# lrmantovani10/Stable-Diffusion.mojo

Hardware: AMD Instinct MI355X
Metric: UNet denoising steps/sec @ 512x512 latent, batch=8 (higher is better)
Workload: dtype f16; 1 GPU; Tiny-SD UNet 512x512 (latent 4x64x64), batch 8/GPU, 50-step DDPM schedule, 77-token context, no CFG, random-init weights (BASELINE configs[1]); global_batch=8, parallelism=dp1 (independent prompts, weights broadcast once)

## Files before the change

### include/tsd.h

```cpp
#ifndef TSD_H
#define TSD_H

#include <stddef.h>
#include <stdint.h>

#ifdef __cplusplus
extern "C" {
#endif

#define TSD_VERSION 100

typedef enum tsd_status {
  TSD_OK = 0,
  TSD_E_ARG = -1,
  TSD_E_SHAPE = -2,
  TSD_E_ALLOC = -3,
  TSD_E_HIP = -4,
  TSD_E_RCCL = -5,
  TSD_E_STATE = -6,
  TSD_E_NONFINITE = -7
} tsd_status;

typedef struct tsd_ctx tsd_ctx;
typedef struct tsd_model tsd_model;
// ... 152 lines not shown
};
#define TSD_GD_VERSION_1 1
enum tsd_gemm_operand { TSD_GO_A0 = 0, TSD_GO_A1, TSD_GO_A2, TSD_GO_W, TSD_GO_WT1, TSD_GO_R, TSD_GO_BIAS, TSD_GO_ROWVEC, TSD_GO_C,
                        TSD_GO_VT, TSD_GO_GN, TSD_GO_COUNT };
int tsd_debug_gemm_record(tsd_ctx* ctx, int on);
int tsd_debug_gemm_recorded(tsd_ctx* ctx, int i, int64_t* desc, int n);
int tsd_debug_gemm_run(tsd_ctx* ctx, const int64_t* desc, int n, int cfg, const void* const* host_in, void* const* host_out,
                       int64_t* ext, int64_t* info);
int tsd_debug_model_fold(tsd_model* m, int block, void* wf, float* bf);
int tsd_debug_attn_bench(tsd_ctx* ctx, int B, int H, int d, int Sq, int Sk, int iters, float* ms);
int tsd_debug_attn_exact_passes(tsd_ctx* ctx, int reset);
int tsd_debug_set_attn_qb(tsd_ctx* ctx, int mode);
int tsd_debug_set_attn_diag(tsd_ctx* ctx, int on);
int tsd_debug_set_res_fuse_skip(tsd_ctx* ctx, int on);
int tsd_debug_set_qkv_fuse(tsd_ctx* ctx, int on);
int tsd_debug_mfma_sustained(tsd_ctx* ctx, float ms_target, float* tflops, float* clock_ghz);

double tsd_flop_count(int kind, int L, int T);

#ifdef __cplusplus
}
#endif
#endif
```

### stable-diffusion.mojo_amd/csrc/api_model.cpp

```cpp
#include <dlfcn.h>
#include <math.h>
#include <string.h>

#include <vector>

#include "graph.h"

#define NOTNULL(p) \
  if (!(p)) TSD_FAIL(TSD_E_ARG, "%s: argument '%s' is NULL", __func__, #p)

namespace {
int h2d(tsd_ctx* c, void* dst, const void* src, size_t bytes) {
  if (c->launch()) HIP_TRY(hipMemcpyAsync(dst, src, bytes, hipMemcpyHostToDevice, c->stream));
  return TSD_OK;
}
int d2h(tsd_ctx* c, void* dst, const void* src, size_t bytes) {
  if (c->launch()) HIP_TRY(hipMemcpyAsync(dst, src, bytes, hipMemcpyDeviceToHost, c->stream));
  return TSD_OK;
}
template <class F>
int run_model(tsd_model* m, F&& fn) {
  tsd_ctx* ctx = m->ctx;
  HIP_TRY(hipSetDevice(ctx->device));
  TSD_TRY(model_check_ready(m));
// ... 90 lines not shown
  tsd_model* dec = nullptr;
  tsd_ctx* ctx = nullptr;
  int B = 0, L = 0, T = 0, Tp = 0, cfg = 0;
  float cfg_scale = 7.5f;
  char* state = nullptr;
  float* latents = nullptr;
  float* lat2 = nullptr;
  half_t* ctx16 = nullptr;
  float* eps = nullptr;
  float* tdev = nullptr;
  float* temb = nullptr;
  float* noise = nullptr;
  float* images = nullptr;
  float* hist = nullptr;
  size_t noise_cap = 0;
  int n_train = 1000, n_infer = 50, start = 0;
  std::vector<float> alphas_cumprod;
  std::vector<int> timesteps;
  int sampler = TSD_SAMPLER_DDPM, spacing = TSD_SPACING_LEADING;
  float eta = 0.f;
  int hist_valid_for = -1;
  bool uploaded = false, has_noise = false;
  size_t plan_unet = 0, plan_dec = 0;
  unsigned opt_gen = 0;
  bool poisoned = false;
  bool decoded = false;
};

static bool host_all_finite(const float* p, size_t n) {
  unsigned bad = 0;
// ... 3 lines not shown
    bad |= ((u & 0x7f800000u) == 0x7f800000u);
  }
  return bad == 0;
}
#define SESSION_NOT_POISONED(s)                                                                                              \
  do {                                                                                                                       \
    if ((s)->poisoned)                                                                                                       \
      TSD_FAIL(TSD_E_NONFINITE, "session: inf / NaN was found in this session's latents or images (reported at an earlier " \
               "download); its state is unusable until upload() replaces it");                                              \
  } while (0)

static int build_schedule(tsd_session* s) {
  sampler_alphas_cumprod(s->n_train, s->alphas_cumprod);
  return sampler_timesteps(s->spacing, s->n_train, s->n_infer, s->start, s->timesteps);
}
static void schedule_changed(tsd_session* s) {
  s->uploaded = false; s->has_noise = false;
  s->hist_valid_for = -1;
  s->decoded = false;
}

extern "C" int tsd_session_create(tsd_model* diffusion, tsd_model* decoder, int B, int L, int T, int cfg,
                                  tsd_session** out) {
  NOTNULL(diffusion); NOTNULL(out);
  if (!is_diffusion_kind(diffusion->kind)) TSD_FAIL(TSD_E_ARG, "session: first model must be a Diffusion");
  if (decoder && (!is_decoder_kind(decoder->kind) || decoder->ctx != diffusion->ctx))
    TSD_FAIL(TSD_E_ARG, "session: decoder must be a Decoder on the same context");
  const int Bu = cfg ? 2 * B : B;
  if (B <= 0 || Bu > 16 || L <= 0 || L % 8 || T <= 0) TSD_FAIL(TSD_E_SHAPE, "session: B=%d (UNet batch %d <= 16) L=%d T=%d", B, Bu, L, T);
  tsd_ctx* ctx = diffusion->ctx;
// ... 14 lines not shown
  s->ctx16 = (half_t*)(s->state + o_ctx); s->eps = (float*)(s->state + o_eps);
  s->tdev = (float*)(s->state + o_t); s->temb = (float*)(s->state + o_te);
  s->images = decoder ? (float*)(s->state + o_img) : nullptr;
  s->hist = (float*)(s->state + o_hist);
  if (build_schedule(s) != TSD_OK) { hipFree(s->state); delete s; return TSD_E_ARG; }
  *out = s;
  return TSD_OK;
}

extern "C" int tsd_session_destroy(tsd_session* s) {
  if (!s) return TSD_OK;
  hipSetDevice(s->ctx->device);
  hipStreamSynchronize(s->ctx->stream);
  if (s->state) hipFree(s->state);
  if (s->noise) hipFree(s->noise);
  delete s;
  return TSD_OK;
}

extern "C" int tsd_session_set_schedule(tsd_session* s, int num_training_steps, int num_inference_steps,
                                        int start_step) {
  NOTNULL(s);
  if (num_training_steps <= 0 || num_inference_steps <= 0 || num_inference_steps > num_training_steps ||
      start_step < 0 || start_step >= num_inference_steps)
    TSD_FAIL(TSD_E_ARG, "schedule: train=%d infer=%d start=%d", num_training_steps, num_inference_steps, start_step);
  s->n_train = num_training_steps; s->n_infer = num_inference_steps; s->start = start_step;
  schedule_changed(s);
  return build_schedule(s);
}
extern "C" int tsd_session_set_sampler(tsd_session* s, int kind, float eta, int spacing) {
// ... 37 lines not shown
    const size_t bytes = s->timesteps.size() * nl * 4;
    if (bytes > s->noise_cap) {
      if (s->noise) HIP_TRY(hipFree(s->noise));
      s->noise = nullptr; s->noise_cap = 0;
      hipError_t e = hipMalloc((void**)&s->noise, bytes);
      if (e != hipSuccess) TSD_FAIL(TSD_E_ALLOC, "session: noise hipMalloc(%zu) failed", bytes);
      s->noise_cap = bytes;
    }
    HIP_TRY(hipMemcpyAsync(s->noise, noise, bytes, hipMemcpyHostToDevice, ctx->stream));
  }
  HIP_TRY(hipStreamSynchronize(ctx->stream));
  TSD_TRY(model_check_ready(s->unet));
  if (s->dec) TSD_TRY(model_check_ready(s->dec));
  Arena& a = ctx->arena;
  const int Bu = s->cfg ? 2 * B : B;
  a.planning = true; a.top = 0; a.peak = 0;
  int r = g_unet_forward(s->unet, s->lat2, s->ctx16, T, Tp, s->temb, Bu, L, s->eps);
  size_t need = a.peak;
  if (r == TSD_OK && s->dec) {
    a.top = 0; a.peak = 0;
    r = g_decoder_forward(s->dec, s->latents, B, L, s->images);
    need = std::max(need, a.peak);
  }
  a.planning = false; a.top = 0; a.peak = 0;
  if (r != TSD_OK) return r;
  TSD_TRY(ctx_reserve_arena(ctx, need));
  s->opt_gen = ctx->opt.gen;
  s->uploaded = true;
  s->poisoned = false;
  s->decoded = false;
  s->hist_valid_for = -1;
  return TSD_OK;
}

static void ddpm_coeffs(const tsd_session* s, int t, int prev, float* sa, float* sb, float* c_x0, float* c_xt, float* sigma) {
  const float a_t = s->alphas_cumprod[t];
  const float a_prev = prev >= 0 ? s->alphas_cumprod[prev] : 1.f;
  const float b_t = 1.f - a_t, b_prev = 1.f - a_prev;
  const float cur_a = a_t / a_prev, cur_b = 1.f - cur_a;
  *sa = sqrtf(a_t); *sb = sqrtf(b_t);
  *c_x0 = sqrtf(a_prev) * cur_b / b_t;
// ... 4 lines not shown
}

extern "C" int tsd_session_step(tsd_session* s, int i) {
  NOTNULL(s);
  if (!s->uploaded) TSD_FAIL(TSD_E_STATE, "session: upload() before step()");
  SESSION_NOT_POISONED(s);
  if (s->opt_gen != s->ctx->opt.gen) TSD_FAIL(TSD_E_STATE, "session: a tsd_debug_set_* call changed this context's options after upload() sized the workspace; upload() again");
  if (i < 0 || i >= (int)s->timesteps.size()) TSD_FAIL(TSD_E_ARG, "session: step %d out of range", i);
  tsd_ctx* ctx = s->ctx;
  const int B = s->B, L = s->L, Bu = s->cfg ? 2 * B : B;
  const size_t nl = (size_t)B * 4 * L * L;
  const int t = s->timesteps[i];
  const bool have_hist = s->sampler == TSD_SAMPLER_DPMPP_2M && s->hist_valid_for == i;
  s->hist_valid_for = -1;
  s->decoded = false;
  TSD_TRY(launch_time_embedding(ctx, nullptr, (float)t, Bu, s->temb));
  const float* lat_in = s->latents;
  if (s->cfg) {
    HIP_TRY(hipMemcpyAsync(s->lat2, s->latents, nl * 4, hipMemcpyDeviceToDevice, ctx->stream));
    HIP_TRY(hipMemcpyAsync(s->lat2 + nl, s->latents, nl * 4, hipMemcpyDeviceToDevice, ctx->stream));
    lat_in = s->lat2;
  }
  ctx->arena.top = 0;
  const bool eps_nhwc = s->unet->unet.final_conv.Opad == 4;
  TSD_TRY(g_unet_forward(s->unet, lat_in, s->ctx16, s->T, s->Tp, s->temb, Bu, L, s->eps, eps_nhwc));
  ctx->arena.top = 0;
  const float* eps_u = s->cfg ? s->eps + nl : nullptr;
  if (s->sampler == TSD_SAMPLER_DDPM) {
    float sa, sb, c_x0, c_xt, sigma;
    const int prev = s->spacing == TSD_SPACING_LEADING ? t - s->n_train / s->n_infer
                                                       : (i + 1 < (int)s->timesteps.size() ? s->timesteps[i + 1] : -1);
    ddpm_coeffs(s, t, prev, &sa, &sb, &c_x0, &c_xt, &sigma);
    const float* nz = (s->has_noise && t > 0) ? s->noise + (size_t)i * nl : nullptr;
    return launch_ddpm_step(ctx, s->latents, s->eps, eps_u, s->cfg_scale, nz, (int64_t)nl, sa, sb, c_x0, c_xt, sigma,
                            eps_nhwc ? L * L : 0);
  }
  double cd[8];
  TSD_TRY(sampler_coeffs(s->sampler, s->eta, s->alphas_cumprod, s->timesteps, i, have_hist ? 1 : 0, cd));
  const SamplerCoeffs c = {(float)cd[2], (float)cd[3], (float)cd[4], (float)cd[5], (float)cd[6], (float)cd[7]};
  const bool multistep = s->sampler == TSD_SAMPLER_DPMPP_2M;
// ... 160 lines not shown
```

### stable-diffusion.mojo_amd/csrc/common.h

```cpp
#pragma once
#include <hip/hip_runtime.h>
#include <stdint.h>
#include <stdio.h>
#include <string>
#include <vector>

#include "../../include/tsd.h"

typedef _Float16 half_t;

void tsd_set_error(const char* fmt, ...);
#define TSD_FAIL(code, ...)      \
  do {                           \
    tsd_set_error(__VA_ARGS__);  \
    return (code);               \
  } while (0)
#define HIP_TRY(expr)                                                                              \
  do {                                                                                             \
    hipError_t e__ = (expr);                                                                       \
    if (e__ != hipSuccess) TSD_FAIL(TSD_E_HIP, "%s failed: %s (%s:%d)", #expr, hipGetErrorString(e__), __FILE__, __LINE__); \
  } while (0)
#define TSD_TRY(expr)            \
  do {                           \
    int r__ = (expr);            \
// ... 11 lines not shown
    size_t n = a + bytes;
    if (n > peak) peak = n;
    if (!planning && n > cap) return nullptr;
    top = n;
    return planning ? (void*)(uintptr_t)(0x1000 + a) : (void*)(base + a);
  }
};

struct TsdOptions {
  int qkv_fuse = 1;
  int res_fuse_skip = 1;
  int gn_composite = 1;
  int conv_in_im2col = 1;
  int chain = 1;
  int fold_out = 1;
  int conv_w_tm_mib = 2, lin_w_tm = 1, lin_w_tm_kib = 1024;
  int attn_qb = 2;
  int attn_qb_force = 0;
  int attn_wg8 = 1;
  int attn8_var = 0;
  int attn_diag = 1;
  int attn_xcd = 0;
  int xcdn = 0, conv_halo = 0, splitk = 1, splitk_mink = 4096, splitk_tiles = 256, splitk_small = 8, splitk_wide = 1, splitk_ring4 = 0,
      splitk_big = 0, sk_cfg = 5, thin_cfg = 0, tune = 15, sk256 = 0, skip128 = 1;
  int force_cfg = -1;
  int sk_big_graph = 0;
  char cfg_override[512] = "";
  int gn_apply_mult = 2;
  int gn_finalize_min = 2048;
  int debug_occ = 0;
// ... 268 lines not shown
```

### stable-diffusion.mojo_amd/csrc/graph.cpp

```cpp
#include <math.h>

#include "graph.h"

#define CHECK_ALLOC(p) \
  if (!(p)) TSD_FAIL(TSD_E_ALLOC, "workspace arena exhausted (%s:%d)", __FILE__, __LINE__)

static int zero_async(tsd_ctx* ctx, void* p, size_t bytes) {
  if (!ctx->launch()) return TSD_OK;
  HIP_TRY(hipMemsetAsync(p, 0, bytes, ctx->stream));
  return TSD_OK;
}

Act act_alloc_gn(tsd_ctx* ctx, int B, int H, int W, int C, int groups) {
  Act a = act_alloc(ctx, B, H, W, C);
  if (a.p && groups > 0 && C % groups == 0) {
    a.gn_buf = arena_alloc<float>(ctx, (int64_t)B * ceil_div(H * W, 32) * groups * 2);
    a.gn_groups = a.gn_buf ? groups : 0;
  }
  return a;
}

static void gn_emit(const tsd_ctx* ctx, GemmArgs& g, Act* dst, int rows_per_sample) {
  if (!dst || !dst->gn_buf || dst->gn_groups <= 0 || g.N != dst->C || (g.epi & (EPI_OUT_F32 | EPI_GEGLU))) return;
  const int ns = gemm_gnstats_slabs(ctx, g.M, g.N, g.K, g.batch, g.conv, rows_per_sample, dst->gn_groups);
// ... 339 lines not shown
  half_t* ao = arena_alloc<half_t>(ctx, M * C); CHECK_ALLOC(ao);
  TSD_TRY(g_qkv_proj(ctx, h0, B, S, C, w.in_proj, qk, vt, S));
  AttnArgs fa;
  fa.Q = qk; fa.ldq = 2 * C; fa.sQ = (int64_t)S * 2 * C;
  fa.K = qk + C; fa.ldk = 2 * C; fa.sK = (int64_t)S * 2 * C;
  fa.Vt = vt; fa.ldvt = S; fa.sVt = (int64_t)C * S;
  fa.O = ao; fa.ldo = C; fa.sO = (int64_t)S * C;
  fa.B = B; fa.H = 1; fa.d = C; fa.Sq = S; fa.Sk = S; fa.scale = 1.f / sqrtf((float)C);
  TSD_TRY(g_attn_core(ctx, fa));
  CatSrc a; a.p0 = ao; a.ld0 = C; a.C0 = C;
  TSD_TRY(g_linear(ctx, a, M, w.out_proj.w, w.out_proj.Kpad, C, C, w.out_proj.b, x.p, x.ld, 0, out.p, out.ld, &out, S));
  ctx->arena.release(mark);
  return TSD_OK;
}

static int g_unet_full_forward(tsd_model* m, const float* latents_chw, const half_t* ctx16, int T, int Tp,
                               const float* temb, int B, int L, float* eps_out_chw, bool eps_nhwc);

int g_unet_forward(tsd_model* m, const float* latents_chw, const half_t* ctx16, int T, int Tp, const float* temb, int B,
                   int L, float* eps_out_chw, bool eps_nhwc) {
  if (is_full_unet_kind(m->kind)) {
    const int prev = gemm_set_splitk_big(m->ctx, 4);
    const int r = g_unet_full_forward(m, latents_chw, ctx16, T, Tp, temb, B, L, eps_out_chw, eps_nhwc);
    gemm_set_splitk_big(m->ctx, prev);
    return r;
  }
  tsd_ctx* ctx = m->ctx;
  const UNetW& u = m->unet;
  if (L % 8) TSD_FAIL(TSD_E_SHAPE, "UNet: latent side %d must be a multiple of 8", L);
  float* t1 = arena_alloc<float>(ctx, (int64_t)B * 1280); CHECK_ALLOC(t1);
  float* time = arena_alloc<float>(ctx, (int64_t)B * 1280); CHECK_ALLOC(time);
  float* tvec = arena_alloc<float>(ctx, (int64_t)B * u.tproj.N); CHECK_ALLOC(tvec);
  TSD_TRY(launch_small_linear(ctx, temb, B, 320, 320, u.t1.w, u.t1.Kpad, u.t1.b, 1280, 0, t1, 1280));
  TSD_TRY(launch_small_linear(ctx, t1, B, 1280, 1280, u.t2.w, u.t2.Kpad, u.t2.b, 1280, 1, time, 1280));
  TSD_TRY(launch_small_linear(ctx, time, B, 1280, 1280, u.tproj.w, u.tproj.Kpad, u.tproj.b, u.tproj.N, 1, tvec,
                              u.tproj.N));
  const int tld = u.tproj.N;
  const bool in_im2col = ctx->opt.conv_in_im2col && u.conv_in_im2col && u.conv1.I == 4;
  Act x0 = act_alloc(ctx, B, L, L, 64); CHECK_ALLOC(x0.p);
  if (in_im2col) TSD_TRY(launch_chw_f32_to_im2col3x3_f16(ctx, latents_chw, B, 4, L, L, x0.p));
  else TSD_TRY(launch_chw_f32_to_nhwc_f16(ctx, latents_chw, B, 4, L, L, 4, 1.f, x0.p, 64));
  Act a[24];
  auto alloc_out = [&](int i, int side, int C) -> int {
    const int groups = i == 23 ? 320 : (i == 11 ? concat_stat_groups(C, 640, 32) : (i == 16 ? concat_stat_groups(C, 320, 32) : 32));
    a[i] = act_alloc_gn(ctx, B, side, side, C, groups);
    CHECK_ALLOC(a[i].p);
    return TSD_OK;
  };
  const int L1 = L / 2, L2 = L / 4;
  auto res = [&](int i, const CatSrc& src, int side_in, int ups) -> int {
    const ResW& w = u.res[i - 1];
    TSD_TRY(alloc_out(i, ups ? side_in * 2 : side_in, w.cout));
    return g_resblock(ctx, src, B, side_in, side_in, ups, w, tvec, tld, a[i]);
  };
  const int CK = u.kproj_all.N;
  half_t* kc_all = arena_alloc<half_t>(ctx, (int64_t)B * Tp * CK); CHECK_ALLOC(kc_all);
  half_t* vtc_all = arena_alloc<half_t>(ctx, (int64_t)B * CK * Tp); CHECK_ALLOC(vtc_all);
  if (ctx_kv_fused_ok(ctx, u, Tp)) {
    GemmArgs g;
    g.A0 = ctx16; g.lda0 = u.kproj_all.Kpad; g.Wt = u.kproj_all.w; g.ldw = u.kproj_all.Kpad;
    g.M = B * Tp; g.N = 2 * CK; g.K = u.kproj_all.Kpad; g.C = kc_all; g.ldc = CK;
    if (u.kproj_all.w_tm) { g.Wt = u.kproj_all.w_tm; g.ldw = 64; g.w_kts = 2 * CK * 128; }
    g.Vt = vtc_all; g.vt_n0 = CK; g.vt_ld = Tp; g.vt_S = Tp; g.vt_sB = (int64_t)CK * Tp;
    TSD_TRY(launch_gemm(ctx, g));
  } else {
    GemmArgs g;
    g.A0 = ctx16; g.lda0 = u.kproj_all.Kpad; g.Wt = u.kproj_all.w; g.ldw = u.kproj_all.Kpad;
    g.M = B * Tp; g.N = CK; g.K = u.kproj_all.Kpad; g.C = kc_all; g.ldc = CK;
    TSD_TRY(launch_gemm(ctx, g));
    GemmArgs v;
    v.A0 = u.vproj_all.w; v.lda0 = u.vproj_all.Kpad; v.sA = 0;
    v.Wt = ctx16; v.ldw = u.vproj_all.Kpad; v.sW = (int64_t)Tp * u.vproj_all.Kpad;
    v.M = CK; v.N = Tp; v.K = u.vproj_all.Kpad; v.batch = B;
    v.C = vtc_all; v.ldc = Tp; v.sC = (int64_t)CK * Tp;
    TSD_TRY(launch_gemm(ctx, v));
  }
  auto attn = [&](int i) -> int {
    TSD_TRY(alloc_out(i, a[i - 1].H, a[i - 1].C));
    const AttnW& w = u.attn[i - 1];
    CtxKV kv;
    kv.K = kc_all + w.kv_off; kv.ldk = CK; kv.sK = (int64_t)Tp * CK;
    kv.Vt = vtc_all + (int64_t)w.kv_off * Tp; kv.ldvt = Tp; kv.sVt = (int64_t)CK * Tp;
    return g_unet_attn(ctx, a[i - 1], w, ctx16, T, Tp, a[i], &kv);
  };
  TSD_TRY(alloc_out(1, L, 320));
  if (in_im2col) TSD_TRY(g_linear(ctx, cat1(x0), (int64_t)B * L * L, u.conv_in_im2col, 64, u.conv1.Opad, 64, u.conv1.b, nullptr, 0, 0, a[1].p,
                                  a[1].ld, &a[1], L * L));
  else TSD_TRY(g_conv3x3(ctx, x0, u.conv1, 1, 1, 1, 0, nullptr, 0, nullptr, 0, false, a[1].p, a[1].ld, &a[1]));
  TSD_TRY(res(2, cat1(a[1]), L, 0));
  TSD_TRY(attn(3));
// ... 19 lines not shown
  TSD_TRY(attn(21));
  TSD_TRY(res(22, cat2(a[21], a[1]), L, 0));
  TSD_TRY(attn(23));
  Act hf = act_alloc(ctx, B, L, L, 320); CHECK_ALLOC(hf.p);
  TSD_TRY(launch_groupnorm(ctx, norm_src(cat1(a[23]), 320), B, L * L, 320, 320, 1e-5f, 1.f, 1, hf.p, hf.ld,
                           a[23].gn_groups == 320 ? a[23].gn_part : nullptr, a[23].gn_nslab));
  if (eps_nhwc && u.final_conv.Opad == 4)
    return g_conv3x3(ctx, hf, u.final_conv, 1, 1, 1, 0, nullptr, 0, nullptr, 0, true, eps_out_chw, 4);
  float* eps_tmp = arena_alloc<float>(ctx, (int64_t)B * L * L * 4); CHECK_ALLOC(eps_tmp);
  TSD_TRY(g_conv3x3(ctx, hf, u.final_conv, 1, 1, 1, 0, nullptr, 0, nullptr, 0, true, eps_tmp, 4));
  TSD_TRY(launch_nhwc_f32_to_chw_f32(ctx, eps_tmp, B, 4, L, L, 4, eps_out_chw));
  return TSD_OK;
}

static int g_unet_full_forward(tsd_model* m, const float* latents_chw, const half_t* ctx16, int T, int Tp,
                               const float* temb, int B, int L, float* eps_out_chw, bool eps_nhwc) {
  tsd_ctx* ctx = m->ctx;
  const UNetW& u = m->unet;
  if (L % 16) TSD_FAIL(TSD_E_SHAPE, "full-size UNet: latent side %d must be a multiple of 16", L);
  float* t1 = arena_alloc<float>(ctx, (int64_t)B * 1280); CHECK_ALLOC(t1);
  float* time = arena_alloc<float>(ctx, (int64_t)B * 1280); CHECK_ALLOC(time);
  float* tvec = arena_alloc<float>(ctx, (int64_t)B * u.tproj.N); CHECK_ALLOC(tvec);
  TSD_TRY(launch_small_linear(ctx, temb, B, 320, 320, u.t1.w, u.t1.Kpad, u.t1.b, 1280, 0, t1, 1280));
  TSD_TRY(launch_small_linear(ctx, t1, B, 1280, 1280, u.t2.w, u.t2.Kpad, u.t2.b, 1280, 1, time, 1280));
  TSD_TRY(launch_small_linear(ctx, time, B, 1280, 1280, u.tproj.w, u.tproj.Kpad, u.tproj.b, u.tproj.N, 1, tvec,
                              u.tproj.N));
  const int tld = u.tproj.N;
  const bool in_im2col = ctx->opt.conv_in_im2col && u.conv_in_im2col && !u.conv.empty() && u.conv[0].I == 4 && SD15_STEPS[0].l.kind == L_CONV &&
                         SD15_STEPS[0].l.d == 1;
  Act x0 = act_alloc(ctx, B, L, L, 64); CHECK_ALLOC(x0.p);
  if (in_im2col) TSD_TRY(launch_chw_f32_to_im2col3x3_f16(ctx, latents_chw, B, 4, L, L, x0.p));
  else TSD_TRY(launch_chw_f32_to_nhwc_f16(ctx, latents_chw, B, 4, L, L, 4, 1.f, x0.p, 64));
  const int CK = u.kproj_all.N;
  half_t* kc_all = arena_alloc<half_t>(ctx, (int64_t)B * Tp * CK); CHECK_ALLOC(kc_all);
  half_t* vtc_all = arena_alloc<half_t>(ctx, (int64_t)B * CK * Tp); CHECK_ALLOC(vtc_all);
  if (ctx_kv_fused_ok(ctx, u, Tp)) {
    GemmArgs g;
    g.A0 = ctx16; g.lda0 = u.kproj_all.Kpad; g.Wt = u.kproj_all.w; g.ldw = u.kproj_all.Kpad;
    g.M = B * Tp; g.N = 2 * CK; g.K = u.kproj_all.Kpad; g.C = kc_all; g.ldc = CK;
    if (u.kproj_all.w_tm) { g.Wt = u.kproj_all.w_tm; g.ldw = 64; g.w_kts = 2 * CK * 128; }
    g.Vt = vtc_all; g.vt_n0 = CK; g.vt_ld = Tp; g.vt_S = Tp; g.vt_sB = (int64_t)CK * Tp;
    TSD_TRY(launch_gemm(ctx, g));
  } else {
    GemmArgs g;
    g.A0 = ctx16; g.lda0 = u.kproj_all.Kpad; g.Wt = u.kproj_all.w; g.ldw = u.kproj_all.Kpad;
    g.M = B * Tp; g.N = CK; g.K = u.kproj_all.Kpad; g.C = kc_all; g.ldc = CK;
    TSD_TRY(launch_gemm(ctx, g));
    GemmArgs v;
    v.A0 = u.vproj_all.w; v.lda0 = u.vproj_all.Kpad; v.sA = 0;
    v.Wt = ctx16; v.ldw = u.vproj_all.Kpad; v.sW = (int64_t)Tp * u.vproj_all.Kpad;
    v.M = CK; v.N = Tp; v.K = u.vproj_all.Kpad; v.batch = B;
    v.C = vtc_all; v.ldc = Tp; v.sC = (int64_t)CK * Tp;
    TSD_TRY(launch_gemm(ctx, v));
  }
  std::vector<Act> skips;
  Act cur = x0;
  for (int i = 0; i < SD15_N; i++) {
    const UNetStep& st = SD15_STEPS[i];
    const LayerDef& l = st.l;
    const int next_groups = i == SD15_N - 1 ? u.final_groups : 32;
    auto stat_groups = [&](int C) -> int {
      if (i + 1 < SD15_N && SD15_STEPS[i + 1].l.kind == L_RES && (SD15_STEPS[i + 1].flags & U_POP) && !(st.flags & U_PUSH) && !skips.empty())
        return concat_stat_groups(C, skips.back().C, 32);
      return next_groups;
    };
    Act y;
    if (l.kind == L_CONV) {
      const int side = cur.H / l.d;
// ... 211 lines not shown
```

### stable-diffusion.mojo_amd/csrc/graph.h

```cpp
#pragma once
#include "model.h"

struct CatSrc {
  const half_t* p0 = nullptr; int ld0 = 0; int C0 = 0;
  const half_t* p1 = nullptr; int ld1 = 0; int C1 = 0;
  const float* gn_part0 = nullptr; int gn_nslab0 = 0, gn_groups0 = 0;
  const float* gn_part1 = nullptr; int gn_nslab1 = 0, gn_groups1 = 0;
};
static inline CatSrc cat1(const Act& a) {
  CatSrc c; c.p0 = a.p; c.ld0 = a.ld; c.C0 = a.C;
  c.gn_part0 = a.gn_part; c.gn_nslab0 = a.gn_nslab; c.gn_groups0 = a.gn_groups;
  return c;
}
static inline int concat_stat_groups(int C0, int C1, int groups) {
  if (C1 <= 0 || C1 % groups || (C0 + C1) % groups) return groups;
  const int cf = C1 / groups, cpg = (C0 + C1) / groups;
  return (cpg % cf == 0 && C0 % cf == 0 && C0 / cf <= 256) ? C0 / cf : groups;
}
Act act_alloc_gn(tsd_ctx* ctx, int B, int H, int W, int C, int groups);
static inline CatSrc cat2(const Act& a, const Act& b) {
  CatSrc c = cat1(a); c.p1 = b.p; c.ld1 = b.ld; c.C1 = b.C;
  c.gn_part1 = b.gn_part; c.gn_nslab1 = b.gn_nslab; c.gn_groups1 = b.gn_groups;
  return c;
}
// ... 6 lines not shown
             const half_t* res, int ldr, int epi_extra, void* y, int ldy, Act* stat = nullptr, int rows_per_sample = 0,
             const half_t* w_tm = nullptr);

int g_resblock(tsd_ctx* ctx, const CatSrc& x, int B, int Hin, int Win, int ups, const ResW& w, const float* tvec,
               int tld, Act& out);
struct CtxKV {
  const half_t* K = nullptr; int ldk = 0; int64_t sK = 0;
  const half_t* Vt = nullptr; int ldvt = 0; int64_t sVt = 0;
};
int g_unet_attn(tsd_ctx* ctx, const Act& x, const AttnW& w, const half_t* ctx16, int T, int Tp, Act& out,
                const CtxKV* pre = nullptr);
int g_vae_attn(tsd_ctx* ctx, const Act& x, const VaeAttnW& w, Act& out);
int g_attn_core(tsd_ctx* ctx, const AttnArgs& fa);
int g_qkv_proj(tsd_ctx* ctx, const half_t* x, int B, int S, int C, const LinW& in_proj, half_t* qk, half_t* vt, int Sp);

int g_unet_forward(tsd_model* m, const float* latents_chw, const half_t* ctx16, int T, int Tp, const float* temb, int B,
                   int L, float* eps_out_chw, bool eps_nhwc = false);
int g_decoder_forward(tsd_model* m, const float* latents_chw, int B, int L, float* images_chw);
int g_encoder_forward(tsd_model* m, const float* images_chw, const float* noise_chw, int B, int S, float* latents_chw);

template <class F>
int run_planned(tsd_ctx* ctx, F&& fn) {
  Arena& a = ctx->arena;
  a.planning = true; a.top = 0; a.peak = 0;
  int r = fn();
  a.planning = false;
  const size_t need = a.peak;
  a.top = 0; a.peak = 0;
  if (r != TSD_OK) return r;
  TSD_TRY(ctx_reserve_arena(ctx, need));
  r = fn();
  a.top = 0;
// ... 4 lines not shown
```

### stable-diffusion.mojo_amd/csrc/model.cpp

```cpp
#include <math.h>
#include <string.h>

#include "model.h"

bool attn_tail_weights_ok(const AttnW& w) {
  const int C = w.C;
  const bool plain = !w.ln[1].w && !w.ln[1].b && !w.ln[2].w && !w.ln[2].b && !w.gelu_erf;
  return plain && C == 320 && w.n_head == 8 && w.n_embed == 40 && w.sa_out.b && w.ca_out.b && w.geglu1.b && w.geglu2.b &&
         w.conv_out.b && !w.ca_q.b && w.sa_out.Kpad == C && w.ca_q.Kpad == C && w.ca_out.Kpad == C && w.geglu1.Kpad == C &&
         w.geglu2.Kpad == 4 * C && w.conv_out.Ipad == C && w.conv_out.k == 1;
}

bool attn_head_weights_ok(const AttnW& w) {
  const int C = w.C;
  return C == 320 && w.n_head == 8 && w.n_embed == 40 && !w.gn.w && !w.gn.b && !w.ln[0].w && !w.ln[0].b && w.conv_in.b &&
         w.conv_in.k == 1 && w.conv_in.Ipad == C && w.conv_in.Opad == C && !w.sa_in.b && w.sa_in.Kpad == C && w.sa_in.N == 3 * C;
}

static void model_invalidate_derived(tsd_model* m) {
  m->ready = false;
  for (auto& a : m->unet.attn) { a.tail_stream = nullptr; a.head_stream = nullptr; a.fold_w = nullptr; a.fold_w_tm = nullptr; a.fold_b = nullptr; }
  m->unet.conv_in_im2col = nullptr;
  m->vae.conv_in_im2col = nullptr;
  for (auto& r : m->unet.res) { r.conv1.w_tm = nullptr; r.conv2.w_tm = nullptr; }
  m->unet.conv4.w_tm = nullptr; m->unet.conv7.w_tm = nullptr; m->unet.kproj_all.w_tm = nullptr;
  for (auto& cv : m->unet.conv) cv.w_tm = nullptr;
  for (auto& a : m->unet.attn) {
    for (LinW* l : {&a.sa_in, &a.sa_out, &a.ca_q, &a.ca_out, &a.geglu1, &a.geglu2}) l->w_tm = nullptr;
    a.conv_in.w_tm = nullptr; a.conv_out.w_tm = nullptr;
  }
}

static size_t packed_bytes(const ParamSpec& p) {
  if (!p.used) return 0;
  switch (p.kind) {
// ... 487 lines not shown
```

### stable-diffusion.mojo_amd/csrc/model.h

```cpp
#pragma once
#include <map>
#include <string>
#include <vector>

#include "common.h"

enum ParamKind { P_CONV_W = 0, P_CONV_B = 1, P_LIN_W = 2, P_LIN_B = 3 };

struct ParamSpec {
  std::string name;
  int64_t shape[4] = {0, 0, 0, 0};
  int ndim = 0;
  int kind = 0;
  bool used = true;
  float bound = 0.f;
  float offset = 0.f;
  int Opad = 0, Kpad = 0;
  int interleave = 0;
  int region = 0;
  size_t off = 0, bytes = 0;
  int64_t numel() const {
    int64_t n = 1;
    for (int i = 0; i < ndim; i++) n *= shape[i];
    return n;
// ... 76 lines not shown
  ClipLayerW layer[12];
  NormAffine final_ln;
};

struct PlanKey { int B, L, T; bool operator<(const PlanKey& o) const { return B != o.B ? B < o.B : (L != o.L ? L < o.L : T < o.T); } };

struct tsd_model {
  tsd_ctx* ctx = nullptr;
  int kind = 0;
  std::vector<ParamSpec> params;
  std::map<std::string, int> index;
  char* blob = nullptr;
  size_t blob_bytes = 0;
  std::vector<char> loaded;
  bool ready = false;
  UNetW unet;
  VaeW vae;
  ClipW clip;
  std::map<PlanKey, size_t> plans;
  char* derived = nullptr;
  size_t derived_bytes = 0;
};

int model_resolve(tsd_model* m);
ConvW model_conv(const tsd_model* m, const std::string& prefix);
LinW model_lin(const tsd_model* m, const std::string& prefix, bool use_bias);
int model_check_ready(tsd_model* m);
```

### stable-diffusion.mojo_amd/csrc/runtime.cpp

```cpp
#include <stdarg.h>
#include <stdlib.h>
#include <string.h>

#include "common.h"

static thread_local char g_err[512] = "";

void tsd_set_error(const char* fmt, ...) {
  va_list ap;
  va_start(ap, fmt);
  vsnprintf(g_err, sizeof(g_err), fmt, ap);
  va_end(ap);
}

static int env_int(const char* name, int dflt) { const char* e = getenv(name); return e && *e ? atoi(e) : dflt; }
void options_from_env(TsdOptions& o) {
  o.qkv_fuse = env_int("TSD_QKV_FUSE", o.qkv_fuse);
  o.res_fuse_skip = env_int("TSD_RES_FUSE_SKIP", o.res_fuse_skip);
  o.gn_composite = env_int("TSD_GN_COMPOSITE", o.gn_composite);
  o.conv_in_im2col = env_int("TSD_CONV_IN_IM2COL", o.conv_in_im2col);
  o.chain = env_int("TSD_CHAIN", o.chain) ? 1 : 0;
  o.fold_out = env_int("TSD_FOLD_OUT", o.fold_out) ? 1 : 0;
  o.conv_w_tm_mib = env_int("TSD_CONV_W_TM", o.conv_w_tm_mib);
  o.lin_w_tm = env_int("TSD_LIN_W_TM", o.lin_w_tm);
  o.lin_w_tm_kib = env_int("TSD_LIN_W_TM_KIB", o.lin_w_tm_kib);
  { const int q = env_int("TSD_ATTN_QB", o.attn_qb); if (q == 1 || q == 2) o.attn_qb = q; }
  o.attn_xcd = env_int("TSD_ATTN_XCD", o.attn_xcd);
  o.attn_wg8 = env_int("TSD_ATTN_WG8", o.attn_wg8) ? 1 : 0;
  o.attn8_var = env_int("TSD_ATTN8_VAR", o.attn8_var);
  o.xcdn = env_int("TSD_GEMM_XCDN", o.xcdn);
  o.conv_halo = env_int("TSD_CONV_HALO", o.conv_halo);
  o.splitk = env_int("TSD_GEMM_SPLITK", o.splitk);
  o.splitk_mink = env_int("TSD_GEMM_SPLITK_MINK", o.splitk_mink);
  o.splitk_tiles = env_int("TSD_GEMM_SPLITK_TILES", o.splitk_tiles);
  o.splitk_small = env_int("TSD_GEMM_SPLITK_SMALL", o.splitk_small);
  o.splitk_wide = env_int("TSD_GEMM_SPLITK_WIDE", o.splitk_wide);
  o.splitk_ring4 = env_int("TSD_GEMM_SPLITK_RING4", o.splitk_ring4);
// ... 192 lines not shown
```

### stable-diffusion.mojo_amd/tsd/_lib.py

```python
import ctypes as C
import os

import numpy as np

_HERE = os.path.dirname(os.path.abspath(__file__))
LIB_PATH = os.environ.get("TSD_LIB") or os.path.join(os.path.dirname(_HERE), "lib", "libtsd.so")

TSD_OK, TSD_E_ARG, TSD_E_SHAPE, TSD_E_ALLOC, TSD_E_HIP, TSD_E_RCCL, TSD_E_STATE, TSD_E_NONFINITE = 0, -1, -2, -3, -4, -5, -6, -7
os.environ.setdefault("HIP_FORCE_DEV_KERNARG", "1")

MODEL_DIFFUSION, MODEL_DECODER, MODEL_ENCODER, MODEL_CLIP, MODEL_DIFFUSION_SD15, MODEL_DIFFUSION_SD15_TORCH = 1, 2, 3, 4, 5, 6
MODEL_CLIP_TORCH, MODEL_DECODER_TORCH, MODEL_ENCODER_TORCH = 7, 8, 9
SAMPLER_KINDS = {"ddpm": 0, "ddim": 1, "dpmpp_2m": 2}
TIMESTEP_SPACINGS = {"leading": 0, "trailing": 1}


def sampler_kind(kind):
    return SAMPLER_KINDS.get(kind.lower(), -1) if isinstance(kind, str) else int(kind)


def timestep_spacing(spacing):
    return TIMESTEP_SPACINGS.get(spacing.lower(), -1) if isinstance(spacing, str) else int(spacing)


# ... 81 lines not shown
        "tsd_dist_unique_id": ([vp], i), "tsd_dist_init": ([vp, i, i, vp], i),
        "tsd_dist_broadcast_weights": ([vp, i], i), "tsd_dist_finalize": ([vp], i),
        "tsd_dist_comm_count": ([vp, C.POINTER(i)], i),
        "tsd_flop_count": ([i, i, i], C.c_double),
        "tsd_debug_splitk_errors": ([vp], i),
        "tsd_debug_xcd_round_robin": ([], i),
        "tsd_debug_nonfinite_count": ([vp, i], i),
        "tsd_debug_set_fused_attention": ([vp, i], i),
        "tsd_debug_gemm_bench": ([vp, i, i, i, i, i, i, i, i, i, i, fp], i),
        "tsd_debug_attn_bench": ([vp, i, i, i, i, i, i, fp], i),
        "tsd_debug_attn_exact_passes": ([vp, i], i),
        "tsd_debug_set_attn_qb": ([vp, i], i),
        "tsd_debug_set_attn_diag": ([vp, i], i),
        "tsd_debug_set_res_fuse_skip": ([vp, i], i),
        "tsd_debug_set_qkv_fuse": ([vp, i], i),
        "tsd_debug_mfma_sustained": ([vp, C.c_float, fp, fp], i),
        "tsd_debug_gemm_check": ([vp, i, i, i, i, i, i, i, i, i, i, fp, fp], i),
        "tsd_debug_gemm_record": ([vp, i], i),
        "tsd_debug_gemm_recorded": ([vp, i, C.POINTER(i64), i], i),
        "tsd_debug_model_fold": ([vp, i, vp, fp], i),
        "tsd_debug_gemm_run": ([vp, C.POINTER(i64), i, i, C.POINTER(vp), C.POINTER(vp), C.POINTER(i64), C.POINTER(i64)], i),
    }
    for name, (args, res) in sig.items():
        fn = getattr(l, name)
        fn.argtypes = args
        fn.restype = res


EXPORTS = None

# ... 95 lines not shown
```

### stable-diffusion.mojo_amd/tsd/model.py

```python
import ctypes as C

import numpy as np

from . import _lib
from ._lib import check, f32, lib, ptr, sampler_kind, timestep_spacing, vp

KINDS = {"diffusion": _lib.MODEL_DIFFUSION, "decoder": _lib.MODEL_DECODER, "encoder": _lib.MODEL_ENCODER,
         "clip": _lib.MODEL_CLIP, "diffusion_sd15": _lib.MODEL_DIFFUSION_SD15,
         "diffusion_sd15_torch": _lib.MODEL_DIFFUSION_SD15_TORCH, "clip_torch": _lib.MODEL_CLIP_TORCH,
         "decoder_torch": _lib.MODEL_DECODER_TORCH, "encoder_torch": _lib.MODEL_ENCODER_TORCH}


def param_specs(kind):
    k = KINDS[kind] if isinstance(kind, str) else kind
    n = lib().tsd_model_param_count(k)
    out = []
    name = C.create_string_buffer(128)
    shape = (C.c_int64 * 4)()
    ndim, used, bound = C.c_int(), C.c_int(), C.c_float()
    for i in range(n):
        check(lib().tsd_model_param_info(k, i, name, 128, shape, C.byref(ndim), C.byref(used), C.byref(bound)))
        out.append((name.value.decode(), tuple(int(shape[j]) for j in range(ndim.value)), bool(used.value), bound.value))
    return out

# ... 97 lines not shown
        check(lib().tsd_session_add_noise(self.h, int(i), ptr(f32(noise))))

    def decode(self):
        check(lib().tsd_session_decode(self.h))

    def latents(self):
        out = np.empty((self.B, 4, self.L, self.L), dtype=np.float32)
        check(lib().tsd_session_download_latents(self.h, ptr(out)))
        return out

    def images(self, rescale=True):
        out = np.empty((self.B, 3, 8 * self.L, 8 * self.L), dtype=np.float32)
        check(lib().tsd_session_download_images(self.h, 1 if rescale else 0, ptr(out)))
        return out

    def close(self):
        if self.h:
            lib().tsd_session_destroy(self.h)
            self.h = None
```

Before: 211.1 steps/s.

## Hoist step-invariant context K/V and time-embedding MLP out of UNet step

At upload time the session now precomputes the cross-attention context K/V projections and a per-timestep table of time-embedding MLP outputs into dedicated device buffers. Each denoising step then passes these through a UNetPre struct instead of recomputing the K/V GEMMs and three small linears. The goal is to remove per-step launches and GEMM work that is constant across steps. The cost is extra device memory, an upfront build at upload, and gen-counter tracking so weight changes trigger a rebuild.

```diff
diff --git a/include/tsd.h b/include/tsd.h
--- a/include/tsd.h
+++ b/include/tsd.h
@@ -190,6 +190,8 @@
 int tsd_debug_set_attn_diag(tsd_ctx* ctx, int on);
 int tsd_debug_set_res_fuse_skip(tsd_ctx* ctx, int on);
 int tsd_debug_set_qkv_fuse(tsd_ctx* ctx, int on);
+int tsd_debug_set_session_hoist(tsd_ctx* ctx, int on);
+int tsd_debug_session_hoist_info(tsd_session* s, int64_t* info);
 int tsd_debug_mfma_sustained(tsd_ctx* ctx, float ms_target, float* tflops, float* clock_ghz);
 
 double tsd_flop_count(int kind, int L, int T);
diff --git a/stable-diffusion.mojo_amd/csrc/api_model.cpp b/stable-diffusion.mojo_amd/csrc/api_model.cpp
--- a/stable-diffusion.mojo_amd/csrc/api_model.cpp
+++ b/stable-diffusion.mojo_amd/csrc/api_model.cpp
@@ -1,5 +1,6 @@
 #include <dlfcn.h>
 #include <math.h>
+#include <stdint.h>
 #include <string.h>
 
 #include <vector>
@@ -128,6 +129,14 @@
   float* images = nullptr;
   float* hist = nullptr;
   size_t noise_cap = 0;
+  char* kv = nullptr;
+  half_t* kc_all = nullptr;
+  half_t* vtc_all = nullptr;
+  float* ttab = nullptr;
+  size_t kv_cap = 0, ttab_cap = 0;
+  bool hoist = false;
+  unsigned model_gen = 0;
+  int inv_builds = 0;
   int n_train = 1000, n_infer = 50, start = 0;
   std::vector<float> alphas_cumprod;
   std::vector<int> timesteps;
@@ -161,6 +170,40 @@
   sampler_alphas_cumprod(s->n_train, s->alphas_cumprod);
   return sampler_timesteps(s->spacing, s->n_train, s->n_infer, s->start, s->timesteps);
 }
+static int session_build_invariants(tsd_session* s) {
+  tsd_ctx* ctx = s->ctx;
+  tsd_model* m = s->unet;
+  const int Bu = s->cfg ? 2 * s->B : s->B, N = m->unet.tproj.N;
+  ctx->arena.top = 0;
+  TSD_TRY(g_unet_ctx_kv(m, s->ctx16, s->Tp, Bu, s->kc_all, s->vtc_all));
+  for (size_t i = 0; i < s->timesteps.size(); i++) {
+    ctx->arena.top = 0;
+    TSD_TRY(launch_time_embedding(ctx, nullptr, (float)s->timesteps[i], Bu, s->temb));
+    const float* tvec = nullptr;
+    TSD_TRY(g_unet_time_path(m, s->temb, Bu, &tvec));
+    HIP_TRY(hipMemcpyAsync(s->ttab + i * (size_t)N, tvec, (size_t)N * 4, hipMemcpyDeviceToDevice, ctx->stream));
+  }
+  ctx->arena.top = 0;
+  s->model_gen = m->gen;
+  s->inv_builds++;
+  return TSD_OK;
+}
+static UNetPre session_pre(const tsd_session* s, int i) {
+  UNetPre p;
+  p.tvec = s->ttab + (size_t)i * s->unet->unet.tproj.N; p.tld = 0;
+  p.kc_all = s->kc_all; p.vtc_all = s->vtc_all;
+  return p;
+}
+extern "C" int tsd_debug_set_session_hoist(tsd_ctx* ctx, int on) {
+  return ctx_set_option(ctx, &TsdOptions::session_hoist, on ? 1 : 0, 0, 1);
+}
+extern "C" int tsd_debug_session_hoist_info(tsd_session* s, int64_t* info) {
+  NOTNULL(s); NOTNULL(info);
+  info[0] = s->uploaded && s->hoist; info[1] = (int64_t)(uintptr_t)s->ttab; info[2] = (int64_t)(uintptr_t)s->kc_all;
+  info[3] = (int64_t)(uintptr_t)s->vtc_all; info[4] = (int64_t)(s->kv_cap + s->ttab_cap); info[5] = s->inv_builds;
+  return TSD_OK;
+}
+
 static void schedule_changed(tsd_session* s) {
   s->uploaded = false; s->has_noise = false;
   s->hist_valid_for = -1;
@@ -205,6 +248,8 @@
   hipStreamSynchronize(s->ctx->stream);
   if (s->state) hipFree(s->state);
   if (s->noise) hipFree(s->noise);
+  if (s->kv) hipFree(s->kv);
+  if (s->ttab) hipFree(s->ttab);
   delete s;
   return TSD_OK;
 }
@@ -272,9 +317,36 @@
   if (s->dec) TSD_TRY(model_check_ready(s->dec));
   Arena& a = ctx->arena;
   const int Bu = s->cfg ? 2 * B : B;
+  s->hoist = ctx->opt.session_hoist != 0;
+  s->uploaded = false;
+  if (s->hoist) {
+    const int CK = s->unet->unet.kproj_all.N, N = s->unet->unet.tproj.N;
+    const size_t kc_bytes = ((size_t)Bu * Tp * CK * 2 + 255) & ~size_t(255), kv_bytes = 2 * kc_bytes;
+    const size_t tt_bytes = s->timesteps.size() * (size_t)N * 4;
+    if (kv_bytes > s->kv_cap) {
+      if (s->kv) HIP_TRY(hipFree(s->kv));
+      s->kv = nullptr; s->kv_cap = 0;
+      if (hipMalloc((void**)&s->kv, kv_bytes) != hipSuccess) TSD_FAIL(TSD_E_ALLOC, "session: context K/V hipMalloc(%zu) failed", kv_bytes);
+      s->kv_cap = kv_bytes;
+    }
+    s->kc_all = (half_t*)s->kv; s->vtc_all = (half_t*)(s->kv + kc_bytes);
+    if (tt_bytes > s->ttab_cap) {
+      if (s->ttab) HIP_TRY(hipFree(s->ttab));
+      s->ttab = nullptr; s->ttab_cap = 0;
+      if (hipMalloc((void**)&s->ttab, tt_bytes) != hipSuccess) TSD_FAIL(TSD_E_ALLOC, "session: time table hipMalloc(%zu) failed", tt_bytes);
+      s->ttab_cap = tt_bytes;
+    }
+  }
   a.planning = true; a.top = 0; a.peak = 0;
-  int r = g_unet_forward(s->unet, s->lat2, s->ctx16, T, Tp, s->temb, Bu, L, s->eps);
+  const UNetPre pre0 = s->hoist ? session_pre(s, 0) : UNetPre();
+  int r = g_unet_forward(s->unet, s->lat2, s->ctx16, T, Tp, s->temb, Bu, L, s->eps, false, s->hoist ? &pre0 : nullptr);
   size_t need = a.peak;
+  if (r == TSD_OK && s->hoist) {
+    const float* tv = nullptr;
+    a.top = 0; a.peak = 0;
+    r = g_unet_time_path(s->unet, s->temb, Bu, &tv);
+    need = std::max(need, a.peak);
+  }
   if (r == TSD_OK && s->dec) {
     a.top = 0; a.peak = 0;
     r = g_decoder_forward(s->dec, s->latents, B, L, s->images);
@@ -283,6 +355,8 @@
   a.planning = false; a.top = 0; a.peak = 0;
   if (r != TSD_OK) return r;
   TSD_TRY(ctx_reserve_arena(ctx, need));
+  s->model_gen = s->unet->gen;
+  if (s->hoist) TSD_TRY(session_build_invariants(s));
   s->opt_gen = ctx->opt.gen;
   s->uploaded = true;
   s->poisoned = false;
@@ -317,7 +391,12 @@
   const bool have_hist = s->sampler == TSD_SAMPLER_DPMPP_2M && s->hist_valid_for == i;
   s->hist_valid_for = -1;
   s->decoded = false;
-  TSD_TRY(launch_time_embedding(ctx, nullptr, (float)t, Bu, s->temb));
+  if (s->model_gen != s->unet->gen) {
+    TSD_TRY(model_check_ready(s->unet));
+    if (s->hoist) TSD_TRY(session_build_invariants(s));
+    s->model_gen = s->unet->gen;
+  }
+  if (!s->hoist) TSD_TRY(launch_time_embedding(ctx, nullptr, (float)t, Bu, s->temb));
   const float* lat_in = s->latents;
   if (s->cfg) {
     HIP_TRY(hipMemcpyAsync(s->lat2, s->latents, nl * 4, hipMemcpyDeviceToDevice, ctx->stream));
@@ -326,7 +405,8 @@
   }
   ctx->arena.top = 0;
   const bool eps_nhwc = s->unet->unet.final_conv.Opad == 4;
-  TSD_TRY(g_unet_forward(s->unet, lat_in, s->ctx16, s->T, s->Tp, s->temb, Bu, L, s->eps, eps_nhwc));
+  const UNetPre pre = s->hoist ? session_pre(s, i) : UNetPre();
+  TSD_TRY(g_unet_forward(s->unet, lat_in, s->ctx16, s->T, s->Tp, s->temb, Bu, L, s->eps, eps_nhwc, s->hoist ? &pre : nullptr));
   ctx->arena.top = 0;
   const float* eps_u = s->cfg ? s->eps + nl : nullptr;
   if (s->sampler == TSD_SAMPLER_DDPM) {
diff --git a/stable-diffusion.mojo_amd/csrc/common.h b/stable-diffusion.mojo_amd/csrc/common.h
--- a/stable-diffusion.mojo_amd/csrc/common.h
+++ b/stable-diffusion.mojo_amd/csrc/common.h
@@ -49,6 +49,7 @@
   int conv_in_im2col = 1;
   int chain = 1;
   int fold_out = 1;
+  int session_hoist = 1;
   int conv_w_tm_mib = 2, lin_w_tm = 1, lin_w_tm_kib = 1024;
   int attn_qb = 2;
   int attn_qb_force = 0;
diff --git a/stable-diffusion.mojo_amd/csrc/graph.cpp b/stable-diffusion.mojo_amd/csrc/graph.cpp
--- a/stable-diffusion.mojo_amd/csrc/graph.cpp
+++ b/stable-diffusion.mojo_amd/csrc/graph.cpp
@@ -377,20 +377,9 @@
   return TSD_OK;
 }
 
-static int g_unet_full_forward(tsd_model* m, const float* latents_chw, const half_t* ctx16, int T, int Tp,
-                               const float* temb, int B, int L, float* eps_out_chw, bool eps_nhwc);
-
-int g_unet_forward(tsd_model* m, const float* latents_chw, const half_t* ctx16, int T, int Tp, const float* temb, int B,
-                   int L, float* eps_out_chw, bool eps_nhwc) {
-  if (is_full_unet_kind(m->kind)) {
-    const int prev = gemm_set_splitk_big(m->ctx, 4);
-    const int r = g_unet_full_forward(m, latents_chw, ctx16, T, Tp, temb, B, L, eps_out_chw, eps_nhwc);
-    gemm_set_splitk_big(m->ctx, prev);
-    return r;
-  }
+int g_unet_time_path(tsd_model* m, const float* temb, int B, const float** tvec_out) {
   tsd_ctx* ctx = m->ctx;
   const UNetW& u = m->unet;
-  if (L % 8) TSD_FAIL(TSD_E_SHAPE, "UNet: latent side %d must be a multiple of 8", L);
   float* t1 = arena_alloc<float>(ctx, (int64_t)B * 1280); CHECK_ALLOC(t1);
   float* time = arena_alloc<float>(ctx, (int64_t)B * 1280); CHECK_ALLOC(time);
   float* tvec = arena_alloc<float>(ctx, (int64_t)B * u.tproj.N); CHECK_ALLOC(tvec);
@@ -398,7 +387,53 @@
   TSD_TRY(launch_small_linear(ctx, t1, B, 1280, 1280, u.t2.w, u.t2.Kpad, u.t2.b, 1280, 1, time, 1280));
   TSD_TRY(launch_small_linear(ctx, time, B, 1280, 1280, u.tproj.w, u.tproj.Kpad, u.tproj.b, u.tproj.N, 1, tvec,
                               u.tproj.N));
-  const int tld = u.tproj.N;
+  *tvec_out = tvec;
+  return TSD_OK;
+}
+
+int g_unet_ctx_kv(tsd_model* m, const half_t* ctx16, int Tp, int B, half_t* kc_all, half_t* vtc_all) {
+  tsd_ctx* ctx = m->ctx;
+  const UNetW& u = m->unet;
+  const int CK = u.kproj_all.N;
+  if (ctx_kv_fused_ok(ctx, u, Tp)) {
+    GemmArgs g;
+    g.A0 = ctx16; g.lda0 = u.kproj_all.Kpad; g.Wt = u.kproj_all.w; g.ldw = u.kproj_all.Kpad;
+    g.M = B * Tp; g.N = 2 * CK; g.K = u.kproj_all.Kpad; g.C = kc_all; g.ldc = CK;
+    if (u.kproj_all.w_tm) { g.Wt = u.kproj_all.w_tm; g.ldw = 64; g.w_kts = 2 * CK * 128; }
+    g.Vt = vtc_all; g.vt_n0 = CK; g.vt_ld = Tp; g.vt_S = Tp; g.vt_sB = (int64_t)CK * Tp;
+    TSD_TRY(launch_gemm(ctx, g));
+  } else {
+    GemmArgs g;
+    g.A0 = ctx16; g.lda0 = u.kproj_all.Kpad; g.Wt = u.kproj_all.w; g.ldw = u.kproj_all.Kpad;
+    g.M = B * Tp; g.N = CK; g.K = u.kproj_all.Kpad; g.C = kc_all; g.ldc = CK;
+    TSD_TRY(launch_gemm(ctx, g));
+    GemmArgs v;
+    v.A0 = u.vproj_all.w; v.lda0 = u.vproj_all.Kpad; v.sA = 0;
+    v.Wt = ctx16; v.ldw = u.vproj_all.Kpad; v.sW = (int64_t)Tp * u.vproj_all.Kpad;
+    v.M = CK; v.N = Tp; v.K = u.vproj_all.Kpad; v.batch = B;
+    v.C = vtc_all; v.ldc = Tp; v.sC = (int64_t)CK * Tp;
+    TSD_TRY(launch_gemm(ctx, v));
+  }
+  return TSD_OK;
+}
+
+static int g_unet_full_forward(tsd_model* m, const float* latents_chw, const half_t* ctx16, int T, int Tp,
+                               const float* temb, int B, int L, float* eps_out_chw, bool eps_nhwc, const UNetPre* pre);
+
+int g_unet_forward(tsd_model* m, const float* latents_chw, const half_t* ctx16, int T, int Tp, const float* temb, int B,
+                   int L, float* eps_out_chw, bool eps_nhwc, const UNetPre* pre) {
+  if (is_full_unet_kind(m->kind)) {
+    const int prev = gemm_set_splitk_big(m->ctx, 4);
+    const int r = g_unet_full_forward(m, latents_chw, ctx16, T, Tp, temb, B, L, eps_out_chw, eps_nhwc, pre);
+    gemm_set_splitk_big(m->ctx, prev);
+    return r;
+  }
+  tsd_ctx* ctx = m->ctx;
+  const UNetW& u = m->unet;
+  if (L % 8) TSD_FAIL(TSD_E_SHAPE, "UNet: latent side %d must be a multiple of 8", L);
+  const float* tvec = pre ? pre->tvec : nullptr;
+  const int tld = pre ? pre->tld : u.tproj.N;
+  if (!pre) TSD_TRY(g_unet_time_path(m, temb, B, &tvec));
   const bool in_im2col = ctx->opt.conv_in_im2col && u.conv_in_im2col && u.conv1.I == 4;
   Act x0 = act_alloc(ctx, B, L, L, 64); CHECK_ALLOC(x0.p);
   if (in_im2col) TSD_TRY(launch_chw_f32_to_im2col3x3_f16(ctx, latents_chw, B, 4, L, L, x0.p));
@@ -417,26 +452,13 @@
     return g_resblock(ctx, src, B, side_in, side_in, ups, w, tvec, tld, a[i]);
   };
   const int CK = u.kproj_all.N;
-  half_t* kc_all = arena_alloc<half_t>(ctx, (int64_t)B * Tp * CK); CHECK_ALLOC(kc_all);
-  half_t* vtc_all = arena_alloc<half_t>(ctx, (int64_t)B * CK * Tp); CHECK_ALLOC(vtc_all);
-  if (ctx_kv_fused_ok(ctx, u, Tp)) {
-    GemmArgs g;
-    g.A0 = ctx16; g.lda0 = u.kproj_all.Kpad; g.Wt = u.kproj_all.w; g.ldw = u.kproj_all.Kpad;
-    g.M = B * Tp; g.N = 2 * CK; g.K = u.kproj_all.Kpad; g.C = kc_all; g.ldc = CK;
-    if (u.kproj_all.w_tm) { g.Wt = u.kproj_all.w_tm; g.ldw = 64; g.w_kts = 2 * CK * 128; }
-    g.Vt = vtc_all; g.vt_n0 = CK; g.vt_ld = Tp; g.vt_S = Tp; g.vt_sB = (int64_t)CK * Tp;
-    TSD_TRY(launch_gemm(ctx, g));
-  } else {
-    GemmArgs g;
-    g.A0 = ctx16; g.lda0 = u.kproj_all.Kpad; g.Wt = u.kproj_all.w; g.ldw = u.kproj_all.Kpad;
-    g.M = B * Tp; g.N = CK; g.K = u.kproj_all.Kpad; g.C = kc_all; g.ldc = CK;
-    TSD_TRY(launch_gemm(ctx, g));
-    GemmArgs v;
-    v.A0 = u.vproj_all.w; v.lda0 = u.vproj_all.Kpad; v.sA = 0;
-    v.Wt = ctx16; v.ldw = u.vproj_all.Kpad; v.sW = (int64_t)Tp * u.vproj_all.Kpad;
-    v.M = CK; v.N = Tp; v.K = u.vproj_all.Kpad; v.batch = B;
-    v.C = vtc_all; v.ldc = Tp; v.sC = (int64_t)CK * Tp;
-    TSD_TRY(launch_gemm(ctx, v));
+  const half_t* kc_all = pre ? pre->kc_all : nullptr;
+  const half_t* vtc_all = pre ? pre->vtc_all : nullptr;
+  if (!pre) {
+    half_t* kc = arena_alloc<half_t>(ctx, (int64_t)B * Tp * CK); CHECK_ALLOC(kc);
+    half_t* vtc = arena_alloc<half_t>(ctx, (int64_t)B * CK * Tp); CHECK_ALLOC(vtc);
+    TSD_TRY(g_unet_ctx_kv(m, ctx16, Tp, B, kc, vtc));
+    kc_all = kc; vtc_all = vtc;
   }
   auto attn = [&](int i) -> int {
     TSD_TRY(alloc_out(i, a[i - 1].H, a[i - 1].C));
@@ -486,44 +508,26 @@
 }
 
 static int g_unet_full_forward(tsd_model* m, const float* latents_chw, const half_t* ctx16, int T, int Tp,
-                               const float* temb, int B, int L, float* eps_out_chw, bool eps_nhwc) {
+                               const float* temb, int B, int L, float* eps_out_chw, bool eps_nhwc, const UNetPre* pre) {
   tsd_ctx* ctx = m->ctx;
   const UNetW& u = m->unet;
   if (L % 16) TSD_FAIL(TSD_E_SHAPE, "full-size UNet: latent side %d must be a multiple of 16", L);
-  float* t1 = arena_alloc<float>(ctx, (int64_t)B * 1280); CHECK_ALLOC(t1);
-  float* time = arena_alloc<float>(ctx, (int64_t)B * 1280); CHECK_ALLOC(time);
-  float* tvec = arena_alloc<float>(ctx, (int64_t)B * u.tproj.N); CHECK_ALLOC(tvec);
-  TSD_TRY(launch_small_linear(ctx, temb, B, 320, 320, u.t1.w, u.t1.Kpad, u.t1.b, 1280, 0, t1, 1280));
-  TSD_TRY(launch_small_linear(ctx, t1, B, 1280, 1280, u.t2.w, u.t2.Kpad, u.t2.b, 1280, 1, time, 1280));
-  TSD_TRY(launch_small_linear(ctx, time, B, 1280, 1280, u.tproj.w, u.tproj.Kpad, u.tproj.b, u.tproj.N, 1, tvec,
-                              u.tproj.N));
-  const int tld = u.tproj.N;
+  const float* tvec = pre ? pre->tvec : nullptr;
+  const int tld = pre ? pre->tld : u.tproj.N;
+  if (!pre) TSD_TRY(g_unet_time_path(m, temb, B, &tvec));
   const bool in_im2col = ctx->opt.conv_in_im2col && u.conv_in_im2col && !u.conv.empty() && u.conv[0].I == 4 && SD15_STEPS[0].l.kind == L_CONV &&
                          SD15_STEPS[0].l.d == 1;
   Act x0 = act_alloc(ctx, B, L, L, 64); CHECK_ALLOC(x0.p);
   if (in_im2col) TSD_TRY(launch_chw_f32_to_im2col3x3_f16(ctx, latents_chw, B, 4, L, L, x0.p));
   else TSD_TRY(launch_chw_f32_to_nhwc_f16(ctx, latents_chw, B, 4, L, L, 4, 1.f, x0.p, 64));
   const int CK = u.kproj_all.N;
-  half_t* kc_all = arena_alloc<half_t>(ctx, (int64_t)B * Tp * CK); CHECK_ALLOC(kc_all);
-  half_t* vtc_all = arena_alloc<half_t>(ctx, (int64_t)B * CK * Tp); CHECK_ALLOC(vtc_all);
-  if (ctx_kv_fused_ok(ctx, u, Tp)) {
-    GemmArgs g;
-    g.A0 = ctx16; g.lda0 = u.kproj_all.Kpad; g.Wt = u.kproj_all.w; g.ldw = u.kproj_all.Kpad;
-    g.M = B * Tp; g.N = 2 * CK; g.K = u.kproj_all.Kpad; g.C = kc_all; g.ldc = CK;
-    if (u.kproj_all.w_tm) { g.Wt = u.kproj_all.w_tm; g.ldw = 64; g.w_kts = 2 * CK * 128; }
-    g.Vt = vtc_all; g.vt_n0 = CK; g.vt_ld = Tp; g.vt_S = Tp; g.vt_sB = (int64_t)CK * Tp;
-    TSD_TRY(launch_gemm(ctx, g));
-  } else {
-    GemmArgs g;
-    g.A0 = ctx16; g.lda0 = u.kproj_all.Kpad; g.Wt = u.kproj_all.w; g.ldw = u.kproj_all.Kpad;
-    g.M = B * Tp; g.N = CK; g.K = u.kproj_all.Kpad; g.C = kc_all; g.ldc = CK;
-    TSD_TRY(launch_gemm(ctx, g));
-    GemmArgs v;
-    v.A0 = u.vproj_all.w; v.lda0 = u.vproj_all.Kpad; v.sA = 0;
-    v.Wt = ctx16; v.ldw = u.vproj_all.Kpad; v.sW = (int64_t)Tp * u.vproj_all.Kpad;
-    v.M = CK; v.N = Tp; v.K = u.vproj_all.Kpad; v.batch = B;
-    v.C = vtc_all; v.ldc = Tp; v.sC = (int64_t)CK * Tp;
-    TSD_TRY(launch_gemm(ctx, v));
+  const half_t* kc_all = pre ? pre->kc_all : nullptr;
+  const half_t* vtc_all = pre ? pre->vtc_all : nullptr;
+  if (!pre) {
+    half_t* kc = arena_alloc<half_t>(ctx, (int64_t)B * Tp * CK); CHECK_ALLOC(kc);
+    half_t* vtc = arena_alloc<half_t>(ctx, (int64_t)B * CK * Tp); CHECK_ALLOC(vtc);
+    TSD_TRY(g_unet_ctx_kv(m, ctx16, Tp, B, kc, vtc));
+    kc_all = kc; vtc_all = vtc;
   }
   std::vector<Act> skips;
   Act cur = x0;
diff --git a/stable-diffusion.mojo_amd/csrc/graph.h b/stable-diffusion.mojo_amd/csrc/graph.h
--- a/stable-diffusion.mojo_amd/csrc/graph.h
+++ b/stable-diffusion.mojo_amd/csrc/graph.h
@@ -44,8 +44,15 @@
 int g_attn_core(tsd_ctx* ctx, const AttnArgs& fa);
 int g_qkv_proj(tsd_ctx* ctx, const half_t* x, int B, int S, int C, const LinW& in_proj, half_t* qk, half_t* vt, int Sp);
 
+struct UNetPre {
+  const float* tvec = nullptr; int tld = 0;
+  const half_t* kc_all = nullptr;
+  const half_t* vtc_all = nullptr;
+};
 int g_unet_forward(tsd_model* m, const float* latents_chw, const half_t* ctx16, int T, int Tp, const float* temb, int B,
-                   int L, float* eps_out_chw, bool eps_nhwc = false);
+                   int L, float* eps_out_chw, bool eps_nhwc = false, const UNetPre* pre = nullptr);
+int g_unet_time_path(tsd_model* m, const float* temb, int B, const float** tvec_out);
+int g_unet_ctx_kv(tsd_model* m, const half_t* ctx16, int Tp, int B, half_t* kc_all, half_t* vtc_all);
 int g_decoder_forward(tsd_model* m, const float* latents_chw, int B, int L, float* images_chw);
 int g_encoder_forward(tsd_model* m, const float* images_chw, const float* noise_chw, int B, int S, float* latents_chw);
 
diff --git a/stable-diffusion.mojo_amd/csrc/model.cpp b/stable-diffusion.mojo_amd/csrc/model.cpp
--- a/stable-diffusion.mojo_amd/csrc/model.cpp
+++ b/stable-diffusion.mojo_amd/csrc/model.cpp
@@ -19,6 +19,7 @@
 
 static void model_invalidate_derived(tsd_model* m) {
   m->ready = false;
+  m->gen++;
   for (auto& a : m->unet.attn) { a.tail_stream = nullptr; a.head_stream = nullptr; a.fold_w = nullptr; a.fold_w_tm = nullptr; a.fold_b = nullptr; }
   m->unet.conv_in_im2col = nullptr;
   m->vae.conv_in_im2col = nullptr;
diff --git a/stable-diffusion.mojo_amd/csrc/model.h b/stable-diffusion.mojo_amd/csrc/model.h
--- a/stable-diffusion.mojo_amd/csrc/model.h
+++ b/stable-diffusion.mojo_amd/csrc/model.h
@@ -114,6 +114,7 @@
   size_t blob_bytes = 0;
   std::vector<char> loaded;
   bool ready = false;
+  unsigned gen = 0;
   UNetW unet;
   VaeW vae;
   ClipW clip;
diff --git a/stable-diffusion.mojo_amd/csrc/runtime.cpp b/stable-diffusion.mojo_amd/csrc/runtime.cpp
--- a/stable-diffusion.mojo_amd/csrc/runtime.cpp
+++ b/stable-diffusion.mojo_amd/csrc/runtime.cpp
@@ -21,6 +21,7 @@
   o.conv_in_im2col = env_int("TSD_CONV_IN_IM2COL", o.conv_in_im2col);
   o.chain = env_int("TSD_CHAIN", o.chain) ? 1 : 0;
   o.fold_out = env_int("TSD_FOLD_OUT", o.fold_out) ? 1 : 0;
+  o.session_hoist = env_int("TSD_SESSION_HOIST", o.session_hoist) ? 1 : 0;
   o.conv_w_tm_mib = env_int("TSD_CONV_W_TM", o.conv_w_tm_mib);
   o.lin_w_tm = env_int("TSD_LIN_W_TM", o.lin_w_tm);
   o.lin_w_tm_kib = env_int("TSD_LIN_W_TM_KIB", o.lin_w_tm_kib);
diff --git a/stable-diffusion.mojo_amd/tsd/_lib.py b/stable-diffusion.mojo_amd/tsd/_lib.py
--- a/stable-diffusion.mojo_amd/tsd/_lib.py
+++ b/stable-diffusion.mojo_amd/tsd/_lib.py
@@ -119,6 +119,8 @@
         "tsd_debug_set_attn_diag": ([vp, i], i),
         "tsd_debug_set_res_fuse_skip": ([vp, i], i),
         "tsd_debug_set_qkv_fuse": ([vp, i], i),
+        "tsd_debug_set_session_hoist": ([vp, i], i),
+        "tsd_debug_session_hoist_info": ([vp, C.POINTER(i64)], i),
         "tsd_debug_mfma_sustained": ([vp, C.c_float, fp, fp], i),
         "tsd_debug_gemm_check": ([vp, i, i, i, i, i, i, i, i, i, i, fp, fp], i),
         "tsd_debug_gemm_record": ([vp, i], i),
diff --git a/stable-diffusion.mojo_amd/tsd/model.py b/stable-diffusion.mojo_amd/tsd/model.py
--- a/stable-diffusion.mojo_amd/tsd/model.py
+++ b/stable-diffusion.mojo_amd/tsd/model.py
@@ -135,6 +135,11 @@
         check(lib().tsd_session_download_images(self.h, 1 if rescale else 0, ptr(out)))
         return out
 
+    def hoist_info(self):
+        info = (C.c_int64 * 6)()
+        check(lib().tsd_debug_session_hoist_info(self.h, info))
+        return dict(zip(("active", "time_table", "ctx_k", "ctx_vt", "bytes", "builds"), (int(v) for v in info)))
+
     def close(self):
         if self.h:
             lib().tsd_session_destroy(self.h)
```

New measurement: 214.0 steps/s (median of 6 runs). 1.01x the previous value.
